# AndrewCullacino/handwritten-chinese-ocr-samples

Measured on AMD Instinct MI355X. Metric: text-lines/sec (1x128x2000 synth) greedy decode, higher is better.
Workload: dtype f16 (f32 accumulate); 1 GPU; BASELINE configs[1]: 64 x 1x128x2000 uint8 lines, random-init hctr checkpoint (C=7358), forward + greedy CTC decode, labels to host; global_lines=64, lines_per_gpu=64, width=2000, classes=7358, checkpoint=random, parallelism=batch-shard x1

## Files before the change

### handwritten-chinese-ocr-samples_amd/_lib.py

```python
import ctypes
import os
import subprocess
import sys

PKG_DIR = os.path.dirname(os.path.abspath(__file__))
ROOT = os.path.dirname(PKG_DIR)
CSRC = os.path.join(PKG_DIR, "csrc")
LIB_PATH = os.path.join(PKG_DIR, "libhctr_hip.so")
HEADER = os.path.join(ROOT, "include", "hctr_hip.h")

SOURCES = [("gather.cpp", ["-x", "hip"]), ("kernels.hip", []), ("preprocess.hip", ["-ffp-contract=off"]), ("engine.cpp", ["-x", "hip"]), ("beam_search.cpp", ["-ffp-contract=off"]),
           ("ngram_lm.cpp", ["-ffp-contract=off"])]
COMMON = ["--offload-arch=gfx950", "-O3", "-std=c++17", "-fPIC", "-Wall", "-Wno-unused-function"]

HCTR_OK = 0
ERR_ARG, ERR_HIP, ERR_STATE, ERR_KEY, ERR_SHAPE, ERR_EMPTY_LINE, ERR_NOMEM = -1, -2, -3, -4, -5, -6, -7
U8, F32, I64 = 0, 1, 2


def _headers():
    return [os.path.join(CSRC, "kernels.h"), os.path.join(CSRC, "ngram_lm.h"), os.path.join(CSRC, "lm_flat.h"), HEADER]


def _deps():
    return [os.path.join(CSRC, s) for s, _ in SOURCES] + _headers()


def source_hash():
    import hashlib
    h = hashlib.sha256()
    h.update(repr((COMMON, SOURCES)).encode())
    for d in sorted(_deps()):
        h.update(os.path.basename(d).encode())
        with open(d, "rb") as f:
            h.update(f.read())
    return h.hexdigest()[:16]


_MARK = b"hctr-src="


def embedded_hash(path=None):
    path = path or LIB_PATH
    try:
# ... 137 lines not shown
    ("hctr_nbest_skip_logits", _I, [_VP, _VP, _VP, _I, _I, _I, _I, _I, _I, ctypes.c_double, ctypes.c_double, _VP, _VP, _VP,
                                    _VP, _VP, _VP, _VP, _VP, _VP]),
    ("hctr_nbest_skip", _I, [_VP, _VP, _VP, _I, _I, _VP, _I, _I, _I, _I, ctypes.c_double, ctypes.c_double, _VP, _VP, _VP,
                             _VP, _VP, _VP, _VP, _VP, _VP]),
    ("hctr_beam_search", _I, [ctypes.POINTER(BeamParams), _I, _I, _I, _I, _VP, _VP, _VP, _VP, _VP, _VP, _VP,
                              _VP, _VP, _VP]),
    ("hctr_ngram_load", _I, [ctypes.c_char_p, ctypes.POINTER(_VP)]),
    ("hctr_ngram_free", None, [_VP]),
    ("hctr_ngram_order", _I, [_VP]),
    ("hctr_ngram_word_id", ctypes.c_int32, [_VP, ctypes.c_char_p]),
    ("hctr_ngram_score", ctypes.c_double, [_VP, ctypes.c_char_p, _I, _I]),
    ("hctr_ngram_word_logp", ctypes.c_double, [_VP, _VP, _I, ctypes.c_int32]),
    ("hctr_ngram_last_error", ctypes.c_char_p, []),
    ("hctr_comm_unique_id", _I, [_VP]),
    ("hctr_comm_create", _I, [ctypes.POINTER(_VP), _VP, _I, _I, _I]),
    ("hctr_comm_destroy", None, [_VP]),
    ("hctr_gather_labels", _I, [_VP, _VP, _VP, _I, _I, _I, _I, _VP, _VP]),
    ("hctr_comm_last_error", ctypes.c_char_p, []),
    ("hctr_resize_lines", _I, [_VP, _VP, _I64, c_i64p, c_i32p, c_i32p, c_i32p, _I, _I, c_i32p, _I, _VP, _I]),
    ("hctr_set_profiling", _I, [_VP, _I]),
    ("hctr_last_profile", _I, [_VP, ctypes.c_char_p, _I, c_f32p, _I]),
    ("hctr_debug_stamps", _I64, [_VP, ctypes.c_char_p, _VP, _I64]),
    ("hctr_debug_activation", _I64, [_VP, ctypes.c_char_p, _VP, _I64, ctypes.POINTER(_I), ctypes.POINTER(_I)]),
]


def load():
    global _LIB
    if _LIB is not None:
        return _LIB
    alt = os.environ.get("HCTR_LIB_PATH", "")
    if alt:
        if not os.path.isfile(alt):
            raise RuntimeError("HCTR_LIB_PATH=%s does not exist" % alt)
    elif _stale():
        try:
            build()
        except FileNotFoundError as exc:
            if not os.path.isfile(LIB_PATH):
                raise RuntimeError("libhctr_hip.so is missing and hipcc is not available (%s); "
                                   "the hctr engine has no CPU fallback" % exc)
            print("hctr: WARNING: sources are newer than libhctr_hip.so but hipcc is not available; "
                  "loading the prebuilt library", file=sys.stderr)
        except (OSError, subprocess.CalledProcessError) as exc:
            raise RuntimeError("libhctr_hip.so is out of date and rebuilding it failed (%s); fix the build "
                               "(python -c 'import hctr_amd; hctr_amd.build(force=True, verbose=True)')" % exc)
    try:
        import torch
    except ImportError:
        pass
    lib = ctypes.CDLL(alt or LIB_PATH)
    if not alt and embedded_hash() != source_hash():
        print("hctr: WARNING: libhctr_hip.so was built from other sources than csrc/ holds now (%s vs %s)"
              % (embedded_hash(), source_hash()), file=sys.stderr)
    host_only = bool(alt) and os.environ.get("HCTR_HOST_ONLY", "") == "1"
    for name, res, args in SIGNATURES:
        if host_only and not hasattr(lib, name):
            continue
        fn = getattr(lib, name)
        fn.restype = res
        fn.argtypes = args
    _LIB = lib
    return lib


_EXC = {ERR_ARG: ValueError, ERR_HIP: RuntimeError, ERR_STATE: RuntimeError, ERR_KEY: KeyError,
        ERR_SHAPE: RuntimeError, ERR_EMPTY_LINE: IndexError, ERR_NOMEM: MemoryError}


def check(rc, ctx=None):
    if rc == HCTR_OK:
        return
    msg = load().hctr_last_error(ctx)
    msg = msg.decode("utf-8", "replace") if msg else ""
    raise _EXC.get(rc, RuntimeError)("hctr engine error %d: %s" % (rc, msg))


def usable_cpus():
    n = len(os.sched_getaffinity(0))
    for path in ("/sys/fs/cgroup/cpu.max",):
        try:
# ... 16 lines not shown
```

### handwritten-chinese-ocr-samples_amd/csrc/engine.cpp

```cpp
#include "../../include/hctr_hip.h"
#include "kernels.h"

#include <algorithm>
#include <cfloat>
#include <cmath>
#include <cstdarg>
#include <cstdio>
#include <cstring>
#include <map>
#include <new>
#include <string>
#include <vector>

using namespace hctr;

namespace {

constexpr int kImgH = 128;
constexpr int kFeat = 2048;
constexpr double kBnEps = 1e-5;
constexpr int kStagePlanes[4] = {128, 256, 512, 512};
constexpr int kStageBlocks[4] = {2, 4, 5, 1};
constexpr int kStageH[5] = {128, 64, 32, 16, 8};
constexpr int64_t kDefaultMaxCols = 131072;

std::string g_create_error;

struct HostTensor {
    std::vector<float> data;
    std::vector<int64_t> shape;
    mutable bool used = false;
};

struct ConvW {
    half_t* w = nullptr;
    float* bias = nullptr;
    int cin = 0, cout = 0, coutPad = 0, taps = 0;
};

struct SeW {
    float* w1 = nullptr;
    float* w2 = nullptr;
    int c = 0;
};

struct BlockW {
    ConvW conv1, conv2, ds;
    SeW se;
    bool has_ds = false;
};

struct Workspace {
    int B = 0, W = 0, Wa = 0;
    void* img = nullptr;
    int32_t* widths = nullptr;
    half_t* s0 = nullptr;
    half_t* x[5] = {};
    half_t* p[5][3] = {};
// ... 258 lines not shown
                    const double v = (double)w->data[((size_t)co * cin + ci) * taps + t] * sc;
                    wmax = std::max(wmax, std::fabs(v));
                    half_t* row = &hw[((size_t)t * coutPad + blk * 64 + s) * cinp];
                    const half_t hi = (half_t)(float)v;
                    row[ci] = hi;
                    if (c->split) {
                        row[cin + ci] = hi;
                        row[2 * cin + ci] = (c->x3_mask & 1) ? (half_t)(float)(v - (double)(float)hi) : (half_t)0.f;
                    }
                }
        }
    for (int co = 0; co < cout; ++co) {
        const double sc = (double)g->data[co] / std::sqrt((double)var->data[co] + kBnEps);
        const double bb = has_bias ? (double)b->data[co] : 0.0;
        hb[co] = (float)((bb - (double)mean->data[co]) * sc + (double)beta->data[co]);
    }
    if (!(wmax < 65000.0))
        return fail(c, HCTR_ERR_ARG, "%s: BatchNorm-folded weight magnitude %.3g does not fit fp16", ck.c_str(), wmax);
    out->cin = cinp; out->cout = cout; out->coutPad = coutPad; out->taps = taps;
    TRY(dev_alloc(c, c->wallocs, &out->w, hw.size(), false));
    TRY(dev_alloc(c, c->wallocs, &out->bias, hb.size(), false));
    HIP_TRY(c, hipMemcpyAsync(out->w, hw.data(), hw.size() * sizeof(half_t), hipMemcpyHostToDevice, c->stream));
    HIP_TRY(c, hipMemcpyAsync(out->bias, hb.data(), hb.size() * sizeof(float), hipMemcpyHostToDevice, c->stream));
    HIP_TRY(c, hipStreamSynchronize(c->stream));
    return HCTR_OK;
}

int build_se(hctr_ctx* c, const std::string& key, int ch, SeW* out) {
    const HostTensor *w1, *w2;
    TRY(need(c, key + ".fc.0.weight", {ch / 16, ch}, &w1));
    TRY(need(c, key + ".fc.2.weight", {ch, ch / 16}, &w2));
    out->c = ch;
    TRY(dev_alloc(c, c->wallocs, &out->w1, w1->data.size(), false));
    TRY(dev_alloc(c, c->wallocs, &out->w2, w2->data.size(), false));
    HIP_TRY(c, hipMemcpyAsync(out->w1, w1->data.data(), w1->data.size() * 4, hipMemcpyHostToDevice, c->stream));
    HIP_TRY(c, hipMemcpyAsync(out->w2, w2->data.data(), w2->data.size() * 4, hipMemcpyHostToDevice, c->stream));
    HIP_TRY(c, hipStreamSynchronize(c->stream));
    return HCTR_OK;
}

int build_stem(hctr_ctx* c, WeightSet& ws) {
    const HostTensor *w, *b, *g, *beta, *mean, *var;
    TRY(need(c, "cnn.conv0_1.weight", {64, 1, 3, 3}, &w));
    TRY(need(c, "cnn.conv0_1.bias", {64}, &b));
    TRY(need(c, "cnn.bn0_1.weight", {64}, &g));
    TRY(need(c, "cnn.bn0_1.bias", {64}, &beta));
// ... 222 lines not shown
    if (c->profiling) { c->prof.clear(); c->ev_used = 0; }
    c->h_widths.clear();
}

struct ActDesc {
    half_t* p;
    int H, C;
};

ConvTile pick_tile(const hctr_ctx* c, const ConvW& cw, int H) {
    if (cw.cout == 64) return TILE_64x256;
    if (c->halo_mode == 2 && cw.taps == 9 && cw.coutPad % 128 == 0 && H % 16 == 0) return TILE_HALO4;
    if (c->halo_mode == 2 && cw.taps == 9 && cw.coutPad % 128 == 0 && H % 8 == 0) return TILE_HALO4_8x32;
    if (c->big_tiles && cw.coutPad % 256 == 0 && H % 16 == 0) return TILE_256x256;
    return TILE_128x128;
}

int run_conv(hctr_ctx* c, Prof& pf, const char* name, const ConvW& cw, ActDesc in, half_t* out, int outH,
             bool relu, bool pool, float* se_part, bool to_head, const float* se_scale = nullptr,
             const half_t* resid = nullptr, const ConvW* ds = nullptr, const half_t* ds_in = nullptr,
             int stem_img_f32 = -1, bool stem_widths = false) {
    const Workspace& ws = c->ws;
    ConvArgs a{};
    a.x = in.p; a.w = cw.w; a.bias = cw.bias; a.y = out; a.se_part = se_part;
    a.se_scale = se_scale; a.resid = resid;
    a.split = c->split ? 1 : 0;
    a.drop_lo = (c->split && !(c->x3_mask & c->out_class)) ? 1 : 0;
    const int m = c->chm();
    a.H = in.H; a.W = ws.W; a.Cin = cw.cin; a.Cout = cw.cout; a.CoutPad = cw.coutPad;
    const ConvTile tile = pick_tile(c, cw, in.H);
    const int rows = conv_tile_rows(tile);
    if (in.H % rows != 0 || cw.cin % kBK != 0)
        return fail(c, HCTR_ERR_ARG, "conv %s: H=%d or Cin=%d not tileable", name, in.H, cw.cin);
    const int cols = conv_tile_cols(tile);
    a.tilesW = (ws.W + cols - 1) / cols;
    a.tilesH = in.H / rows;
    a.in_sb = (int64_t)(in.H + 2) * ws.Wa * cw.cin;
    a.in_sh = ws.Wa * cw.cin;
    if (a.in_sb * 2 >= ((int64_t)1 << 32) || (int64_t)(outH + 2) * ws.Wa * cw.cout * m * 2 >= ((int64_t)1 << 32))
        return fail(c, HCTR_ERR_ARG, "line width %d too large: one image's activation exceeds the kernels' 32-bit "
                    "in-image byte offsets (conv %s)", ws.W, name);
    if (to_head) {
        a.out_sb = (int64_t)ws.W * kFeat * m; a.out_sh = 512 * m; a.out_sw = kFeat * m; a.out_off = 0;
        a.out_wlimit = ws.W;
    } else {
        a.out_sb = (int64_t)(outH + 2) * ws.Wa * cw.cout * m;
        a.out_sh = ws.Wa * cw.cout * m; a.out_sw = cw.cout * m;
// ... 2314 lines not shown
            } else {
                L.mode = 2;
            }
        }
        HIP_TRY(c, hipSetDevice(c->device));
        std::vector<void*> tmp;
        PoolGuard tmp_guard{tmp};
        return synced(c, [&]() -> int {
            uint8_t *src = nullptr, *dst = out;
            ResizeLine* dl = nullptr;
            const size_t out_bytes = (size_t)n * out_height * out_W;
            TRY(dev_alloc(c, tmp, &src, (size_t)std::max<int64_t>(packed_bytes, 1), false));
            TRY(dev_alloc(c, tmp, &dl, (size_t)n, false));
            if (!out_on_device) TRY(dev_alloc(c, tmp, &dst, out_bytes, false));
            HIP_TRY(c, hipMemcpyAsync(src, packed_src, (size_t)packed_bytes, hipMemcpyHostToDevice, c->stream));
            HIP_TRY(c, hipMemcpyAsync(dl, lines.data(), sizeof(ResizeLine) * (size_t)n, hipMemcpyHostToDevice, c->stream));
            HIP_TRY(c, launch_resize_lines(src, dl, n, dst, out_height, out_W, c->stream));
            if (!out_on_device) HIP_TRY(c, hipMemcpyAsync(out, dst, out_bytes, hipMemcpyDeviceToHost, c->stream));
            return HCTR_OK;
        }());
    });
}

int64_t hctr_debug_stamps(hctr_ctx* c, const char* layer, uint64_t* out, int64_t cap_wgs) {
    return guard<int64_t>(c, [&]() -> int64_t {
        if (!c || cap_wgs < 0) return HCTR_ERR_ARG;
        if (hipSetDevice(c->device) != hipSuccess) return fail(c, HCTR_ERR_HIP, "hipSetDevice");
        if (layer) {
            if (c->stamp_buf) { (void)hipFree(c->stamp_buf); c->stamp_buf = nullptr; }
            c->stamp_layer = layer;
            c->stamp_cap = cap_wgs;
            c->stamp_n = 0;
            if (cap_wgs > 0 && hipMalloc((void**)&c->stamp_buf, (size_t)cap_wgs * 128) != hipSuccess)
                return fail(c, HCTR_ERR_NOMEM, "stamp buffer");
            return 0;
        }
        if (!out || !c->stamp_buf) return fail(c, HCTR_ERR_STATE, "stamping not armed");
        const int64_t n = std::min(c->stamp_n, cap_wgs);
        if (hipMemcpy(out, c->stamp_buf, (size_t)n * 128, hipMemcpyDeviceToHost) != hipSuccess)
            return fail(c, HCTR_ERR_HIP, "stamp copy");
        return n;
    });
}

int64_t hctr_debug_activation(hctr_ctx* c, const char* name, float* out, int64_t cap, int* Cout, int* Hout) {
    return guard<int64_t>(c, [&]() -> int64_t {
// ... 50 lines not shown
```

### handwritten-chinese-ocr-samples_amd/csrc/kernels.h

```cpp
#pragma once
#include <hip/hip_runtime.h>
#include <stdint.h>

#include "lm_flat.h"

namespace hctr {

typedef _Float16 half_t;

constexpr int kTileW = 16;
constexpr int kBK = 64;

struct ConvArgs {
    const half_t* x;
    const half_t* w;
    const float* bias;
    void* y;
    float* se_part;
    const float* se_scale;
    const half_t* resid;
    int H, W;
    int Cin, Cout, CoutPad;
    int tilesW, tilesH;
    int64_t in_sb;
    int in_sh;
    int64_t out_sb;
    int out_sh, out_sw;
    int64_t out_off;
    int out_wlimit;
    int relu, pool;
    int64_t M;
    int64_t ldo;
    int mtiles, ntiles;
    int nt_shift, th_shift;
    uint64_t tw_magic;
    float* amax_val;
    int32_t* amax_idx;
    float* amax_val2;
// ... 187 lines not shown
```

### handwritten-chinese-ocr-samples_amd/csrc/kernels.hip

```cpp
#include "kernels.h"

#include <algorithm>
#include <cstdlib>

namespace hctr {

typedef _Float16 f16x8 __attribute__((ext_vector_type(8)));
typedef float f32x4 __attribute__((ext_vector_type(4)));
typedef float f32x2 __attribute__((ext_vector_type(2)));
typedef _Float16 f16x2 __attribute__((ext_vector_type(2)));
typedef uint32_t u32x4 __attribute__((ext_vector_type(4)));
typedef void __attribute__((address_space(3))) * lptr_t;

__device__ __forceinline__ void glds16_asm(const char* gsrc, char* lds_dst) {
    const uint32_t lds = (uint32_t)(uintptr_t)((lptr_t)lds_dst);
    uint32_t keep;
    asm volatile("s_mov_b32 %0, m0\n\ts_mov_b32 m0, %2\n\ts_nop 0\n\tglobal_load_lds_dwordx4 %1, off\n\ts_mov_b32 m0, %0"
                 : "=&s"(keep)
                 : "v"(gsrc), "s"(lds)
                 : "memory");
}

template <int CTRL>
__device__ __forceinline__ float dpp_f32(float v) {
// ... 6 lines not shown
__device__ __forceinline__ void glds16_asm_s(const char* sbase, uint32_t voff, char* lds_dst) {
    const uint32_t lds = (uint32_t)(uintptr_t)((lptr_t)lds_dst);
    uint32_t keep;
    asm volatile("s_mov_b32 %0, m0\n\ts_mov_b32 m0, %3\n\ts_nop 0\n\tglobal_load_lds_dwordx4 %1, %2\n\ts_mov_b32 m0, %0"
                 : "=&s"(keep)
                 : "v"(voff), "s"(sbase), "s"(lds)
                 : "memory");
}

__device__ __forceinline__ void glds16x4_asm_s(const char* s0, const char* s1, const char* s2, const char* s3, uint32_t voff,
                                               char* d0, char* d1, char* d2, char* d3) {
    const uint32_t l0 = (uint32_t)(uintptr_t)((lptr_t)d0), l1 = (uint32_t)(uintptr_t)((lptr_t)d1);
    const uint32_t l2 = (uint32_t)(uintptr_t)((lptr_t)d2), l3 = (uint32_t)(uintptr_t)((lptr_t)d3);
    uint32_t keep;
    asm volatile("s_mov_b32 %0, m0\n\t"
                 "s_mov_b32 m0, %6\n\ts_nop 0\n\tglobal_load_lds_dwordx4 %1, %2\n\t"
                 "s_mov_b32 m0, %7\n\ts_nop 0\n\tglobal_load_lds_dwordx4 %1, %3\n\t"
                 "s_mov_b32 m0, %8\n\ts_nop 0\n\tglobal_load_lds_dwordx4 %1, %4\n\t"
                 "s_mov_b32 m0, %9\n\ts_nop 0\n\tglobal_load_lds_dwordx4 %1, %5\n\t"
                 "s_mov_b32 m0, %0"
                 : "=&s"(keep)
                 : "v"(voff), "s"(s0), "s"(s1), "s"(s2), "s"(s3), "s"(l0), "s"(l1), "s"(l2), "s"(l3)
                 : "memory");
}

template <int LSTRIDE>
__device__ __forceinline__ void glds16x4v_asm_s(const char* sbase, uint32_t v0, uint32_t v1, uint32_t v2, uint32_t v3, char* d0) {
    const uint32_t l0 = (uint32_t)(uintptr_t)((lptr_t)d0);
    uint32_t keep;
    asm volatile("s_mov_b32 %0, m0\n\t"
                 "s_mov_b32 m0, %6\n\ts_nop 0\n\tglobal_load_lds_dwordx4 %1, %5\n\t"
                 "s_add_u32 m0, m0, %7\n\ts_nop 0\n\tglobal_load_lds_dwordx4 %2, %5\n\t"
                 "s_add_u32 m0, m0, %7\n\ts_nop 0\n\tglobal_load_lds_dwordx4 %3, %5\n\t"
                 "s_add_u32 m0, m0, %7\n\ts_nop 0\n\tglobal_load_lds_dwordx4 %4, %5\n\t"
                 "s_mov_b32 m0, %0"
                 : "=&s"(keep)
                 : "v"(v0), "v"(v1), "v"(v2), "v"(v3), "s"(sbase), "s"(l0), "i"(LSTRIDE)
                 : "memory", "scc");
}

__device__ __forceinline__ constexpr int acc_cout_offset(int j) { return (j >> 2) * 64 + ((j >> 1) & 1) * 32 + (j & 1) * 4; }

constexpr float kSeScaleFloor = 1e-12f;

template <int WN, int WM, int JT, bool LINEAR, bool SPLIT, bool PRIVATE_RED = false, bool BIAS_DONE = false,
          bool RESID_IN_ACC = false>
// ... 754 lines not shown
                if (g + 2 < 8) read_a(g + 2, ar[(g + 2) % 3]);
                __builtin_amdgcn_sched_barrier(0);
                if (g == 1) { read_b(1, bq[1]); __builtin_amdgcn_sched_barrier(0); }
                __builtin_amdgcn_s_setprio(1);
#pragma unroll
                for (int jj = 0; jj < 2; ++jj)
#pragma unroll
                    for (int n = 0; n < 4; ++n)
                        acc[2 * jp + jj][n] = __builtin_amdgcn_mfma_f32_16x16x32_f16(ar[g % 3][jj], bq[ks][n],
                                                                                    acc[2 * jp + jj][n], 0, 0, 0);
                __builtin_amdgcn_s_setprio(0);
                __builtin_amdgcn_sched_barrier(0);
            }
        }
    }
    asm volatile("s_waitcnt vmcnt(0)" ::: "memory");
    conv_epilogue<WN, WM, JT, false, false>(a, acc, smem, tid, lane, wn, wm, n0, mt, img, th, tw, th * 16 + wm * 4,
                                            tw * 16);
}

namespace halo4_lds {
constexpr int kWeightBuf = 16384;
constexpr int kWeights = 0;
constexpr int kHalo = kWeights + 2 * kWeightBuf;
constexpr int kScratch = kHalo + kHaloBytes;
constexpr int kScratchBytes = 4 * 128 * 4;
constexpr int kHaloTable = kScratch;
constexpr int kHaloTableBytes = 4 * 12 * 8 * 4;
constexpr int kNextTile = kScratch + kScratchBytes;
constexpr int kTotal = kNextTile + 16;
static_assert(kHaloTableBytes <= kScratchBytes, "the halo-offset table fits inside the epilogue scratch it aliases");
static_assert(kNextTile >= kScratch + kScratchBytes, "the next-tile words lie behind the epilogue scratch");
static_assert(kTotal <= 80 * 1024, "two workgroups per CU on 160 KB of LDS");
}

template <int GEOM, bool SPLIT, bool PERSIST, bool STAMP = false, bool DSFUSE = false, bool RESPRE = false>
__global__ __launch_bounds__(256, 2) void conv3x3_halo4_kernel(const ConvArgs a) {
    static_assert(!DSFUSE || !PERSIST, "downsample fusion: non-persistent instances only");
    static_assert(!RESPRE || (!DSFUSE && !PERSIST && !SPLIT), "residual-in-prologue: plain f16 instances only");
    constexpr int WN = 1, WM = 4, JT = 8, BN = 128;
    constexpr int TR = GEOM ? 8 : 16, TC = GEOM ? 32 : 16;
    constexpr int S = TC + 4;
    static_assert((TR + 2) * S * 128 == kHaloBytes, "halo footprint");
    extern __shared__ __attribute__((aligned(16))) char smem[];
    const int tid = threadIdx.x;
    auto stamp = [&](int i) {
        if (STAMP && tid == 0) a.stamps[(size_t)blockIdx.x * 16 + i] = __builtin_amdgcn_s_memrealtime();
    };
    stamp(0);
    const int lane = tid & 63;
    const int wv = __builtin_amdgcn_readfirstlane(tid >> 6);
    const int wm = wv;
    const int cin = a.Cin;
    const int nkc = (a.dbg & 64) ? 0 : cin / kBK;
    const int nk = 9 * nkc;
    constexpr bool kPrefetch = !PERSIST && !STAMP && !RESPRE;
    static_assert(!(kPrefetch && PERSIST), "the halo-offset table aliases the epilogue scratch: one tile per workgroup");
    constexpr int kRing = 3;
    constexpr int kBhalfAt = 1;
    constexpr int kBpreAt = 4;
    constexpr int kEarlyAt = 1;

    {
        const int k0 = a.mtiles, k1 = a.ntiles, k2 = a.tilesW, k3 = a.tilesH, k4 = a.Cin, k5 = a.in_sh, k6 = a.nt_shift,
                  k7 = a.th_shift, k8 = a.CoutPad;
        const uint64_t k9 = a.tw_magic;
        const int64_t k10 = a.in_sb;
        const half_t *k11 = a.x, *k12 = a.w;
        const float* k13 = a.bias;
        asm volatile("" ::"s"(k0), "s"(k1), "s"(k2), "s"(k3), "s"(k4), "s"(k5), "s"(k6), "s"(k7), "s"(k8), "s"(k9), "s"(k10),
                     "s"(k11), "s"(k12), "s"(k13));
    }
    const int total = a.mtiles * a.ntiles;
    const int xcd = blockIdx.x & 7, local = blockIdx.x >> 3;
    const int tq = total >> 3, tr = total & 7;
    const int xbase_lin = xcd < tr ? xcd * (tq + 1) : tr * (tq + 1) + (xcd - tr) * tq;
    const int xcnt = tq + (xcd < tr ? 1 : 0);
    const int nloc = PERSIST ? (int)(gridDim.x >> 3) : 1;
    struct Tile { int n0, mt, img, th, tw; const char* xb; const char* wb; };
    auto tile_at = [&](int idx) {
        Tile t;
        const int lin = xbase_lin + idx;
        int nt, t2, th, img;
        if (a.nt_shift >= 0) { nt = lin & (a.ntiles - 1); t.mt = lin >> a.nt_shift; }
        else { nt = lin % a.ntiles; t.mt = lin / a.ntiles; }
        t.n0 = nt * BN;
        t2 = (int)(((uint64_t)(uint32_t)t.mt * a.tw_magic) >> 40);
        const int tw = t.mt - t2 * a.tilesW;
        if (a.th_shift >= 0) { th = t2 & (a.tilesH - 1); img = t2 >> a.th_shift; }
        else { th = t2 % a.tilesH; img = t2 / a.tilesH; }
        t.img = img; t.th = th; t.tw = tw;
// ... 52 lines not shown
        uint32_t* htab = (uint32_t*)(smem + halo4_lds::kHaloTable);
        if ((lane & 7) == 0) {
            const uint32_t cp0 = (uint32_t)((lane >> 3) & 7) << 4;
#pragma unroll
            for (int r = 0; r < 12; ++r) htab[(wv * 12 + r) * 8 + (lane >> 3)] = hoff[r] - cp0;
        }
    };
    const int hbuf = halo4_lds::kHalo + wrow * (S * 128);
    int bx[3][2];
#pragma unroll
    for (int d = 0; d < 3; ++d) {
        const int u = wcol + c + d;
        const int v0 = u * 128 + (((q ^ (u & 7)) & 7) << 4);
        bx[d][0] = hbuf + v0;
        bx[d][1] = hbuf + (v0 ^ 64);
    }
    auto b_ptrs = [&](int tap, const char*& be, const char*& bo) {
        const int tdy = tap / 3, d = tap - tdy * 3;
        be = smem + bx[d][tdy & 1] + tdy * (S * 128);
        bo = smem + bx[d][(tdy & 1) ^ 1] + tdy * (S * 128);
    };

    Tile cur = tile_at(tidx);
    int kbase = 0;
    bool first = true;

    int tile_no = 0;
    for (;;) {
        const bool has_next = PERSIST && (tnext < xcnt);
        const char* nxb = cur.xb;
        const char* nwb = cur.wb;
        if (has_next) {
            const Tile t = tile_at(tnext);
            nxb = t.xb;
            nwb = t.wb;
        }
        int drawn = 0;
        if (dynamic && tid == 0)
            drawn = 2 * nloc + __hip_atomic_fetch_add(a.tile_counter + xcd, 1, __ATOMIC_RELAXED, __HIP_MEMORY_SCOPE_AGENT);
        f32x4 acc[JT][4];
        f16x8 bq[2][4];
        auto mma_step = [&](const char* wt, const char* be, const char* bo, auto&& stage_next, auto&& after_group,
                            bool have_b0 = false, const char* nbe = nullptr, const char* nbo = nullptr,
                            int bhalf_at = kBhalfAt) {
            f16x8 ar[kRing][2];
            auto read_a = [&](int g, f16x8 (&dst)[2]) {
                const int ks = g >> 2, jp = g & 3;
                const char* base = wt + (ks ? aoff1 : aoff0);
                dst[0] = *(const f16x8*)(base + (2 * jp) * 2048);
                dst[1] = *(const f16x8*)(base + (2 * jp + 1) * 2048);
            };
            auto read_b = [&](int ks, f16x8 (&dst)[4]) {
#pragma unroll
                for (int n = 0; n < 4; ++n)
                    dst[n] = *(const f16x8*)((((n & 1) ^ ks) ? bo : be) + n * (S * 128));
            };
            __builtin_amdgcn_sched_barrier(0);
            if (!have_b0) read_b(0, bq[0]);
            read_a(0, ar[0]);
            __builtin_amdgcn_sched_barrier(0);
#pragma unroll
            for (int g = 1; g < kRing - 1; ++g) read_a(g, ar[g]);
            __builtin_amdgcn_sched_barrier(0);
            stage_next();
            __builtin_amdgcn_sched_barrier(0);
#pragma unroll
            for (int g = 0; g < 8; ++g) {
                const int ks = g >> 2, jp = g & 3;
                if (g + kRing - 1 < 8) read_a(g + kRing - 1, ar[(g + kRing - 1) % kRing]);
                __builtin_amdgcn_sched_barrier(0);
                if (g == bhalf_at) { read_b(1, bq[1]); __builtin_amdgcn_sched_barrier(0); }
#pragma unroll
                for (int jj = 0; jj < 2; ++jj)
#pragma unroll
                    for (int n = 0; n < 4; ++n)
                        acc[2 * jp + jj][n] = __builtin_amdgcn_mfma_f32_16x16x32_f16(
                            ar[g % kRing][jj], bq[ks][n], acc[2 * jp + jj][n], 0, 0, 0);
                if (g == kBpreAt && nbe != nullptr) {
#pragma unroll
                    for (int n = 0; n < 4; ++n) bq[0][n] = *(const f16x8*)(((n & 1) ? nbo : nbe) + n * (S * 128));
                }
                after_group(g);
                __builtin_amdgcn_sched_barrier(0);
            }
        };

        if (DSFUSE) {
            const int dcin = a.ds_cin, nds = dcin / kBK;
            const int tw0 = cur.tw, th0 = cur.th, img0 = cur.img;
            const char* dxb = (const char*)(a.ds_x + img0 * a.ds_in_sb + (int64_t)(th0 * TR) * a.ds_in_sh +
                                            (int64_t)(tw0 * TC) * dcin);
            const char* dwb = (const char*)(a.ds_w + (int64_t)cur.n0 * dcin);
            uint32_t woff_x[4];
            lane_offsets(dcin, a.ds_in_sh, woff_x, true);
            lane_offsets(cin, a.in_sh, woff, false);
            stage_halo(dxb, 0);
            stage_w(dwb, dcin, woff_x, 0, 0, 0);
            __builtin_amdgcn_s_setprio(1);
#pragma unroll
            for (int j = 0; j < JT; ++j)
#pragma unroll
                for (int n = 0; n < 4; ++n) acc[j][n] = (f32x4){0.f, 0.f, 0.f, 0.f};
            __builtin_amdgcn_s_waitcnt(0xc07f);
#pragma unroll 1
            for (int kc = 0; kc < nds; ++kc) {
                asm volatile("s_waitcnt vmcnt(0)" ::: "memory");
                __builtin_amdgcn_s_barrier();
                asm volatile("" ::: "memory");
                const char *be, *bo;
                b_ptrs(4, be, bo);
                mma_step(weight_buf(kc), be, bo, [&] {
                    if (kc + 1 < nds) stage_w(dwb, dcin, woff_x, kc + 1, 0, (kc + 1) & 1);
                    else stage_w(cur.wb, cin, woff, 0, 0, (kc + 1) & 1);
                }, [&](int) {});
                __builtin_amdgcn_s_barrier();
                asm volatile("" ::: "memory");
                if (kc + 1 < nds) {
                    stage_halo(dxb, kc + 1);
                } else {
                    lane_offsets(cin, a.in_sh, woff, true);
                    stage_halo(cur.xb, 0);
                    if (kPrefetch) write_halo_table();
                }
            }
            kbase = nds;
            const float* sc = a.se_scale + (int64_t)img0 * a.Cout + cur.n0 + q * 8;
#pragma unroll
            for (int j = 0; j < JT; ++j) {
                const int o = acc_cout_offset(j);
                const f32x4 bd = *(const f32x4*)(a.ds_bias + cur.n0 + q * 8 + o);
                const f32x4 b2 = *(const f32x4*)(a.bias + cur.n0 + q * 8 + o);
                const f32x4 s4 = *(const f32x4*)(sc + o);
#pragma unroll
                for (int i = 0; i < 4; ++i) {
                    const float inv = __builtin_amdgcn_rcpf(fmaxf(s4[i], kSeScaleFloor));
#pragma unroll
                    for (int n = 0; n < 4; ++n) acc[j][n][i] = fmaf(acc[j][n][i] + bd[i], inv, b2[i]);
                }
            }
        } else {
            if (PERSIST || first) lane_offsets(cin, a.in_sh, woff, true);
            if (first) {
                stage_halo(cur.xb, 0);
                stage_weights(cur.wb, 0, 0, 0);
                if (kPrefetch) write_halo_table();
                first = false;
                if (STAMP) {
                    stamp(1);
                    asm volatile("s_waitcnt vmcnt(0)" ::: "memory");
                    __builtin_amdgcn_s_barrier();
                    stamp(2);
                }
            }
            if (RESPRE) {
                const int w = cur.tw * TC + wcol + c;
                const bool wok = w < a.out_wlimit;
                const half_t* rb = a.resid + a.out_off + cur.img * a.out_sb + (int64_t)w * a.out_sw + cur.n0 + q * 8 +
                                   (int64_t)(cur.th * TR + wrow) * a.out_sh;
                const float* sc = a.se_scale + (int64_t)cur.img * a.Cout + cur.n0 + q * 8;
                f16x8 rlo[JT / 4][4], rhi[JT / 4][4];
#pragma unroll
                for (int cb = 0; cb < JT / 4; ++cb)
#pragma unroll
                    for (int n = 0; n < 4; ++n) {
                        const half_t* r = rb + (int64_t)n * a.out_sh + cb * 64;
                        rlo[cb][n] = wok ? *(const f16x8*)r : (f16x8){0, 0, 0, 0, 0, 0, 0, 0};
                        rhi[cb][n] = wok ? *(const f16x8*)(r + 32) : (f16x8){0, 0, 0, 0, 0, 0, 0, 0};
// ... 5 lines not shown
#pragma unroll
                    for (int i = 0; i < 4; ++i) {
                        const float inv = __builtin_amdgcn_rcpf(fmaxf(s4[i], kSeScaleFloor));
                        const int e = (j & 3) * 4 + i;
#pragma unroll
                        for (int n = 0; n < 4; ++n) {
                            const float r = e < 8 ? (float)rlo[j >> 2][n][e] : (float)rhi[j >> 2][n][e - 8];
                            acc[j][n][i] = fmaf(r, inv, b4[i]);
                        }
                    }
                }
            } else {
#pragma unroll
                for (int j = 0; j < JT; ++j) {
                    const f32x4 b4 = *(const f32x4*)(a.bias + cur.n0 + q * 8 + acc_cout_offset(j));
#pragma unroll
                    for (int n = 0; n < 4; ++n) acc[j][n] = b4;
                }
            }
        }

        __builtin_amdgcn_s_waitcnt(0xc07f);
        __builtin_amdgcn_s_setprio(1);
        for (int kc = 0; kc < nkc; ++kc) {
            const bool next_chunk = kc + 1 < nkc;
#pragma unroll
            for (int tap = 0; tap < 9; ++tap) {
                const int k = kc * 9 + tap;
                asm volatile("s_waitcnt vmcnt(0)" ::: "memory");
                if (!(a.dbg & 1024)) __builtin_amdgcn_s_barrier();
                asm volatile("" ::: "memory");
                const char *be, *bo;
                b_ptrs(tap, be, bo);
                const bool more = k + 1 < nk;
                const bool wrap = tap == 8;
                const int tap1 = more ? (wrap ? 0 : tap + 1) : 0;
                const int kc1 = more ? (wrap ? kc + 1 : kc) : 0;
                const char* wsrc = more ? cur.wb : nwb;
                const char *nbe = nullptr, *nbo = nullptr;
                if (kPrefetch && tap < 8) b_ptrs(tap + 1, nbe, nbo);
                mma_step(weight_buf(kbase + k), be, bo, [&] {
                    if ((more || has_next) && !(a.dbg & 512))
                        stage_weights(wsrc, kc1, tap1, (kbase + k + 1) & 1);
                }, [&](int g) {
                    if (kPrefetch && tap == 8 && g == kEarlyAt && next_chunk) {
                        asm volatile("s_waitcnt lgkmcnt(0)" ::: "memory");
                        __builtin_amdgcn_s_barrier();
                        asm volatile("" ::: "memory");
                        static_assert(kHaloPieces == 45, "halo piece count");
                        const char* hsrc = (next_chunk ? cur.xb + (int64_t)(kc + 1) * (kBK * 2) : nxb);
                        char* d = smem + halo4_lds::kHalo + wv * 1024;
                        int ln = lane;
                        asm volatile("" : "+v"(ln));
                        const uint32_t* hrow = (const uint32_t*)(smem + halo4_lds::kHaloTable) + wv * 96 + (ln >> 3);
                        const uint32_t cpl = (uint32_t)((ln ^ (ln >> 3)) & 7) << 4;
                        uint32_t ho[4];
#pragma unroll
                        for (int r = 0; r < 4; ++r) ho[r] = hrow[r * 8] + cpl;
                        glds16x4v_asm_s<4096>(hsrc, ho[0], ho[1], ho[2], ho[3], d);
#pragma unroll
                        for (int r = 0; r < 4; ++r) ho[r] = hrow[(4 + r) * 8] + cpl;
                        glds16x4v_asm_s<4096>(hsrc, ho[0], ho[1], ho[2], ho[3], d + 4 * 4096);
#pragma unroll
                        for (int r = 0; r < 4; ++r) ho[r] = hrow[(8 + r) * 8] + cpl;
#pragma unroll
                        for (int r = 8; r < 11; ++r) glds16_asm_s(hsrc, ho[r - 8], d + r * 4096);
                        if (wv == 0) glds16_asm_s(hsrc, ho[3], d + 11 * 4096);
                    }
                }, kPrefetch && tap > 0, nbe, nbo, (kPrefetch && tap == 8) ? 0 : kBhalfAt);
            }
            if (!kPrefetch && (next_chunk || has_next) && !(a.dbg & 32)) {
                __builtin_amdgcn_s_barrier();
                asm volatile("" ::: "memory");
                if (next_chunk) stage_halo(cur.xb, kc + 1);
                else stage_halo(nxb, 0);
            }
        }
        __builtin_amdgcn_s_setprio(0);
        stamp(3);
        if (a.dbg & 128) {
            float t = 0.f;
#pragma unroll
            for (int j = 0; j < JT; ++j)
#pragma unroll
                for (int n = 0; n < 4; ++n) t += acc[j][n][0] + acc[j][n][1] + acc[j][n][2] + acc[j][n][3];
            if (t == 123.456f) ((half_t*)a.y)[0] = (half_t)t;
        } else
        {
            const int tw = cur.tw, th = cur.th, img = cur.img;
            conv_epilogue<WN, WM, JT, false, SPLIT, true, true, DSFUSE || RESPRE>(
                a, acc, smem + halo4_lds::kScratch, tid, lane, 0, wm, cur.n0, cur.mt, img, th, tw, th * TR + wrow,
                tw * TC + wcol, STAMP ? a.stamps + (size_t)blockIdx.x * 16 : nullptr);
        }
        if (!has_next) break;
// ... 187 lines not shown
            }
        }
    }
    __builtin_amdgcn_s_setprio(0);
    conv_epilogue<WN, WM, JT, false, false, true, true, false>(a, acc, smem + halo4_lds::kScratch, tid, lane, 0, wm, n0, mt, img, th, tw,
                                                               th * TR + wrow, tw * TC + wcol);
}

template <auto KERNEL>
static hipError_t launch_halo4_instance(const ConvArgs& a0, int grid, hipStream_t s, bool with_env_dbg = true) {
    static bool done[64] = {};
    hipError_t e0 = raise_lds_limit((const void*)KERNEL, halo4_lds::kTotal, done);
    if (e0 != hipSuccess) return e0;
    static const int dbg = env_dbg();
    ConvArgs a = a0;
    if (with_env_dbg) a.dbg |= dbg;
    hipLaunchKernelGGL(KERNEL, dim3(grid), dim3(256), halo4_lds::kTotal, s, a);
    return hipGetLastError();
}

template <int GEOM, bool SPLIT, bool PERSIST>
static hipError_t launch_conv_halo4_tp(const ConvArgs& a, hipStream_t s) {
    int grid = a.mtiles * a.ntiles;
    if (PERSIST) {
        static int cus[64] = {};
        int dev = 0;
        (void)hipGetDevice(&dev);
        if (dev >= 0 && dev < 64 && cus[dev] == 0) {
            hipDeviceProp_t prop;
            if (hipGetDeviceProperties(&prop, dev) == hipSuccess) cus[dev] = prop.multiProcessorCount;
            if (cus[dev] <= 0) cus[dev] = 256;
        }
        const int resident = 2 * ((dev >= 0 && dev < 64) ? cus[dev] : 256);
        if (grid > resident) grid = resident;
        grid = (grid + 7) / 8 * 8;
    }
    return launch_halo4_instance<conv3x3_halo4_kernel<GEOM, SPLIT, PERSIST>>(a, grid, s);
}
template <int GEOM, bool SPLIT>
static hipError_t launch_conv_halo4_t(const ConvArgs& a, hipStream_t s) {
    const int grid = a.mtiles * a.ntiles;
    if (a.ds_x != nullptr) {
        if (GEOM != 0) return hipErrorInvalidValue;
        return launch_halo4_instance<conv3x3_halo4_kernel<0, SPLIT, false, false, true>>(a, grid, s);
    }
    if (a.stamps != nullptr && !SPLIT)
        return launch_halo4_instance<conv3x3_halo4_kernel<GEOM, false, false, true>>(a, grid, s, false);
    static const int persist = [] { const char* e = getenv("HCTR_PERSIST"); return e ? atoi(e) : 0; }();
    if constexpr (!SPLIT) {
        static const int respre = [] { const char* e = getenv("HCTR_RESPRE"); return e ? atoi(e) : 0; }();
        if (respre && persist == 0 && a.resid != nullptr && a.se_scale != nullptr)
            return launch_halo4_instance<conv3x3_halo4_kernel<GEOM, false, false, false, false, true>>(a, grid, s);
    }
    if (persist == 0 || (persist == 2 && a.tile_counter == nullptr)) return launch_conv_halo4_tp<GEOM, SPLIT, false>(a, s);
    ConvArgs b = a;
    if (persist != 2) b.tile_counter = nullptr;
    return launch_conv_halo4_tp<GEOM, SPLIT, true>(b, s);
}
template <int GEOM>
static hipError_t launch_conv_halo4(const ConvArgs& a0, hipStream_t s) {
    ConvArgs a = a0;
    auto shift_of = [](int v) { int sft = 0; while ((1 << sft) < v) ++sft; return (1 << sft) == v ? sft : -1; };
    a.nt_shift = shift_of(a.ntiles);
    a.th_shift = shift_of(a.tilesH);
    if (a.tilesW < 1 || (uint64_t)a.mtiles * (uint64_t)a.tilesW >= ((uint64_t)1 << 40)) return hipErrorInvalidValue;
    a.tw_magic = (((uint64_t)1 << 40) + (uint64_t)a.tilesW - 1) / (uint64_t)a.tilesW;
// ... 2853 lines not shown
```

### include/hctr_hip.h

```cpp
#ifndef HCTR_HIP_H
#define HCTR_HIP_H

#include <stdint.h>

#ifdef __cplusplus
extern "C" {
#endif

typedef struct hctr_ctx hctr_ctx;

typedef enum {
    HCTR_OK = 0,
    HCTR_ERR_ARG = -1,
    HCTR_ERR_HIP = -2,
    HCTR_ERR_STATE = -3,
    HCTR_ERR_KEY = -4,
    HCTR_ERR_SHAPE = -5,
    HCTR_ERR_EMPTY_LINE = -6,
    HCTR_ERR_NOMEM = -7
} hctr_status;

typedef enum { HCTR_U8 = 0, HCTR_F32 = 1, HCTR_I64 = 2 } hctr_dtype;

int hctr_create(hctr_ctx** out, int device, int num_classes);
// ... 164 lines not shown

int hctr_resize_lines(hctr_ctx* ctx, const uint8_t* packed_src, int64_t packed_bytes, const int64_t* offsets,
                      const int32_t* heights, const int32_t* widths, const int32_t* channels, int n,
                      int out_height, const int32_t* out_widths, int out_W, uint8_t* out, int out_on_device);

#define HCTR_COMM_ID_BYTES 128
typedef struct hctr_comm hctr_comm;
int hctr_comm_unique_id(void* id128);
int hctr_comm_create(hctr_comm** out, const void* id128, int rank, int world, int device);
void hctr_comm_destroy(hctr_comm* comm);
int hctr_gather_labels(hctr_comm* comm, const int32_t* labels, const int32_t* lengths, int n_local, int row_stride,
                       int lines_per_rank, int cap, int32_t* out_labels, int32_t* out_lengths);
const char* hctr_comm_last_error(void);

int hctr_set_profiling(hctr_ctx* ctx, int enabled);
int hctr_last_profile(hctr_ctx* ctx, char* names_buf, int cap, float* ms, int max_n);
int hctr_workspace_stats(hctr_ctx* ctx, int64_t* arena_bytes, int64_t* arena_allocations, int64_t* recarves);
int hctr_lines_per_pass(hctr_ctx* ctx, int B, int W, int f16x3);
int64_t hctr_debug_stamps(hctr_ctx* ctx, const char* layer, uint64_t* out, int64_t cap_wgs);

int64_t hctr_debug_activation(hctr_ctx* ctx, const char* name, float* out, int64_t cap,
                              int* C, int* H);

#ifdef __cplusplus
}
#endif
#endif
```

Before: 524.9 lines/s.

## Pre-pack 3x3 conv weights into MFMA-order stream with 4-slot LDS ring

Adds a host-side repack of 3x3 conv weights into a lane-ordered stream layout matching the MFMA operand fragments. The non-persistent halo4 conv kernel can then stage weights with contiguous global_load_lds copies into a four-slot LDS ring, issuing half-tap units at two points per step. This replaces the strided per-lane weight staging and its offset math, and should allow finer-grained overlap of weight loads with MFMA work. The cost is a second device copy of every 3x3 weight. Launches now fail if the packed weights are missing, and the prefetch path is split into a separate loop.

New measurement: 529.3 lines/s, median of 6. Within noise of the previous version (+0.8%).

```diff
diff --git a/handwritten-chinese-ocr-samples_amd/_lib.py b/handwritten-chinese-ocr-samples_amd/_lib.py
--- a/handwritten-chinese-ocr-samples_amd/_lib.py
+++ b/handwritten-chinese-ocr-samples_amd/_lib.py
@@ -19,7 +19,8 @@
 
 
 def _headers():
-    return [os.path.join(CSRC, "kernels.h"), os.path.join(CSRC, "ngram_lm.h"), os.path.join(CSRC, "lm_flat.h"), HEADER]
+    return [os.path.join(CSRC, "kernels.h"), os.path.join(CSRC, "ngram_lm.h"), os.path.join(CSRC, "lm_flat.h"),
+            os.path.join(CSRC, "weight_stream.h"), HEADER]
 
 
 def _deps():
@@ -203,6 +204,7 @@
     ("hctr_last_profile", _I, [_VP, ctypes.c_char_p, _I, c_f32p, _I]),
     ("hctr_debug_stamps", _I64, [_VP, ctypes.c_char_p, _VP, _I64]),
     ("hctr_debug_activation", _I64, [_VP, ctypes.c_char_p, _VP, _I64, ctypes.POINTER(_I), ctypes.POINTER(_I)]),
+    ("hctr_pack_weight_stream", _I, [_VP, _VP, _I, _I, _I, _I]),
 ]
 
 
@@ -238,6 +240,8 @@
     for name, res, args in SIGNATURES:
         if host_only and not hasattr(lib, name):
             continue
+        if alt and name == "hctr_pack_weight_stream" and not hasattr(lib, name):
+            continue
         fn = getattr(lib, name)
         fn.restype = res
         fn.argtypes = args
diff --git a/handwritten-chinese-ocr-samples_amd/csrc/engine.cpp b/handwritten-chinese-ocr-samples_amd/csrc/engine.cpp
--- a/handwritten-chinese-ocr-samples_amd/csrc/engine.cpp
+++ b/handwritten-chinese-ocr-samples_amd/csrc/engine.cpp
@@ -1,5 +1,6 @@
 #include "../../include/hctr_hip.h"
 #include "kernels.h"
+#include "weight_stream.h"
 
 #include <algorithm>
 #include <cfloat>
@@ -34,6 +35,7 @@
 
 struct ConvW {
     half_t* w = nullptr;
+    half_t* ws = nullptr;
     float* bias = nullptr;
     int cin = 0, cout = 0, coutPad = 0, taps = 0;
 };
@@ -338,6 +340,14 @@
     TRY(dev_alloc(c, c->wallocs, &out->bias, hb.size(), false));
     HIP_TRY(c, hipMemcpyAsync(out->w, hw.data(), hw.size() * sizeof(half_t), hipMemcpyHostToDevice, c->stream));
     HIP_TRY(c, hipMemcpyAsync(out->bias, hb.data(), hb.size() * sizeof(float), hipMemcpyHostToDevice, c->stream));
+    std::vector<half_t> hs;
+    if (taps == 9 && wstream::shape_ok(taps, coutPad, cinp)) {
+        static_assert(sizeof(half_t) == sizeof(uint16_t), "fp16 storage");
+        hs.resize(hw.size());
+        wstream::pack((const uint16_t*)hw.data(), (uint16_t*)hs.data(), taps, coutPad, cinp, false);
+        TRY(dev_alloc(c, c->wallocs, &out->ws, hs.size(), false));
+        HIP_TRY(c, hipMemcpyAsync(out->ws, hs.data(), hs.size() * sizeof(half_t), hipMemcpyHostToDevice, c->stream));
+    }
     HIP_TRY(c, hipStreamSynchronize(c->stream));
     return HCTR_OK;
 }
@@ -606,7 +616,7 @@
              int stem_img_f32 = -1, bool stem_widths = false) {
     const Workspace& ws = c->ws;
     ConvArgs a{};
-    a.x = in.p; a.w = cw.w; a.bias = cw.bias; a.y = out; a.se_part = se_part;
+    a.x = in.p; a.w = cw.w; a.ws = cw.ws; a.bias = cw.bias; a.y = out; a.se_part = se_part;
     a.se_scale = se_scale; a.resid = resid;
     a.split = c->split ? 1 : 0;
     a.drop_lo = (c->split && !(c->x3_mask & c->out_class)) ? 1 : 0;
@@ -2967,6 +2977,12 @@
     });
 }
 
+int hctr_pack_weight_stream(const uint16_t* src, uint16_t* dst, int taps, int coutPad, int cin, int inverse) {
+    if (!src || !dst || !wstream::shape_ok(taps, coutPad, cin)) return HCTR_ERR_ARG;
+    wstream::pack(src, dst, taps, coutPad, cin, inverse != 0);
+    return HCTR_OK;
+}
+
 int64_t hctr_debug_stamps(hctr_ctx* c, const char* layer, uint64_t* out, int64_t cap_wgs) {
     return guard<int64_t>(c, [&]() -> int64_t {
         if (!c || cap_wgs < 0) return HCTR_ERR_ARG;
diff --git a/handwritten-chinese-ocr-samples_amd/csrc/kernels.h b/handwritten-chinese-ocr-samples_amd/csrc/kernels.h
--- a/handwritten-chinese-ocr-samples_amd/csrc/kernels.h
+++ b/handwritten-chinese-ocr-samples_amd/csrc/kernels.h
@@ -14,6 +14,7 @@
 struct ConvArgs {
     const half_t* x;
     const half_t* w;
+    const half_t* ws;
     const float* bias;
     void* y;
     float* se_part;
diff --git a/handwritten-chinese-ocr-samples_amd/csrc/kernels.hip b/handwritten-chinese-ocr-samples_amd/csrc/kernels.hip
--- a/handwritten-chinese-ocr-samples_amd/csrc/kernels.hip
+++ b/handwritten-chinese-ocr-samples_amd/csrc/kernels.hip
@@ -52,6 +52,19 @@
                  : "=&s"(keep)
                  : "v"(voff), "s"(s0), "s"(s1), "s"(s2), "s"(s3), "s"(l0), "s"(l1), "s"(l2), "s"(l3)
                  : "memory");
+}
+
+__device__ __forceinline__ void glds16x2_asm_s(const char* s0, uint32_t voff, char* d0) {
+    const char* s1 = s0 + 1024;
+    const uint32_t l0 = (uint32_t)(uintptr_t)((lptr_t)d0);
+    uint32_t keep;
+    asm volatile("s_mov_b32 %0, m0\n\t"
+                 "s_mov_b32 m0, %4\n\ts_nop 0\n\tglobal_load_lds_dwordx4 %1, %2\n\t"
+                 "s_add_u32 m0, m0, 1024\n\ts_nop 0\n\tglobal_load_lds_dwordx4 %1, %3\n\t"
+                 "s_mov_b32 m0, %0"
+                 : "=&s"(keep)
+                 : "v"(voff), "s"(s0), "s"(s1), "s"(l0)
+                 : "memory", "scc");
 }
 
 template <int LSTRIDE>
@@ -852,6 +865,9 @@
 namespace halo4_lds {
 constexpr int kWeightBuf = 16384;
 constexpr int kWeights = 0;
+constexpr int kRingSlot = 8192, kRingSlots = 4;
+static_assert(kRingSlots * kRingSlot == 2 * kWeightBuf, "the ring slots are the two weight buffers");
+static_assert(kRingSlot == 8 * 64 * 16, "a unit is eight 16-cout blocks of 64 lanes x 16 bytes");
 constexpr int kHalo = kWeights + 2 * kWeightBuf;
 constexpr int kScratch = kHalo + kHaloBytes;
 constexpr int kScratchBytes = 4 * 128 * 4;
@@ -886,6 +902,7 @@
     const int nk = 9 * nkc;
     constexpr bool kPrefetch = !PERSIST && !STAMP && !RESPRE;
     static_assert(!(kPrefetch && PERSIST), "the halo-offset table aliases the epilogue scratch: one tile per workgroup");
+    constexpr bool kRingW = kPrefetch;
     constexpr int kRing = 3;
     constexpr int kBhalfAt = 1;
     constexpr int kBpreAt = 4;
@@ -896,7 +913,7 @@
                   k7 = a.th_shift, k8 = a.CoutPad;
         const uint64_t k9 = a.tw_magic;
         const int64_t k10 = a.in_sb;
-        const half_t *k11 = a.x, *k12 = a.w;
+        const half_t *k11 = a.x, *k12 = kRingW ? a.ws : a.w;
         const float* k13 = a.bias;
         asm volatile("" ::"s"(k0), "s"(k1), "s"(k2), "s"(k3), "s"(k4), "s"(k5), "s"(k6), "s"(k7), "s"(k8), "s"(k9), "s"(k10),
                      "s"(k11), "s"(k12), "s"(k13));
@@ -995,6 +1012,10 @@
     };
 
     Tile cur = tile_at(tidx);
+    const char* const wsb = kRingW ? (const char*)(a.ws + (int64_t)cur.n0 * 9 * cin) + wv * 2048 : nullptr;
+    char* const wl = smem + halo4_lds::kWeights + wv * 2048;
+    const uint32_t l16 = (uint32_t)lane * 16u;
+    auto stage_unit = [&](const char* src, int slot_off) { glds16x2_asm_s(src, l16, wl + slot_off); };
     int kbase = 0;
     bool first = true;
 
@@ -1013,9 +1034,7 @@
             drawn = 2 * nloc + __hip_atomic_fetch_add(a.tile_counter + xcd, 1, __ATOMIC_RELAXED, __HIP_MEMORY_SCOPE_AGENT);
         f32x4 acc[JT][4];
         f16x8 bq[2][4];
-        auto mma_step = [&](const char* wt, const char* be, const char* bo, auto&& stage_next, auto&& after_group,
-                            bool have_b0 = false, const char* nbe = nullptr, const char* nbo = nullptr,
-                            int bhalf_at = kBhalfAt) {
+        auto mma_step = [&](const char* wt, const char* be, const char* bo, auto&& stage_next) {
             f16x8 ar[kRing][2];
             auto read_a = [&](int g, f16x8 (&dst)[2]) {
                 const int ks = g >> 2, jp = g & 3;
@@ -1029,13 +1048,51 @@
                     dst[n] = *(const f16x8*)((((n & 1) ^ ks) ? bo : be) + n * (S * 128));
             };
             __builtin_amdgcn_sched_barrier(0);
+            read_b(0, bq[0]);
+            read_a(0, ar[0]);
+            __builtin_amdgcn_sched_barrier(0);
+#pragma unroll
+            for (int g = 1; g < kRing - 1; ++g) read_a(g, ar[g]);
+            __builtin_amdgcn_sched_barrier(0);
+            stage_next();
+            __builtin_amdgcn_sched_barrier(0);
+#pragma unroll
+            for (int g = 0; g < 8; ++g) {
+                const int ks = g >> 2, jp = g & 3;
+                if (g + kRing - 1 < 8) read_a(g + kRing - 1, ar[(g + kRing - 1) % kRing]);
+                __builtin_amdgcn_sched_barrier(0);
+                if (g == kBhalfAt) { read_b(1, bq[1]); __builtin_amdgcn_sched_barrier(0); }
+#pragma unroll
+                for (int jj = 0; jj < 2; ++jj)
+#pragma unroll
+                    for (int n = 0; n < 4; ++n)
+                        acc[2 * jp + jj][n] = __builtin_amdgcn_mfma_f32_16x16x32_f16(
+                            ar[g % kRing][jj], bq[ks][n], acc[2 * jp + jj][n], 0, 0, 0);
+                __builtin_amdgcn_sched_barrier(0);
+            }
+        };
+        auto ring_step = [&](const char* wt, const char* be, const char* bo, auto&& issue0, auto&& mid, auto&& issue1,
+                             auto&& after_group, bool have_b0, const char* nbe, const char* nbo, int bhalf_at) {
+            f16x8 ar[kRing][2];
+            auto read_a = [&](int g, f16x8 (&dst)[2]) {
+                const int ks = g >> 2, jp = g & 3;
+                const char* base = wt + ks * halo4_lds::kRingSlot;
+                dst[0] = *(const f16x8*)(base + (2 * jp) * 1024);
+                dst[1] = *(const f16x8*)(base + (2 * jp + 1) * 1024);
+            };
+            auto read_b = [&](int ks, f16x8 (&dst)[4]) {
+#pragma unroll
+                for (int n = 0; n < 4; ++n)
+                    dst[n] = *(const f16x8*)((((n & 1) ^ ks) ? bo : be) + n * (S * 128));
+            };
+            __builtin_amdgcn_sched_barrier(0);
             if (!have_b0) read_b(0, bq[0]);
             read_a(0, ar[0]);
             __builtin_amdgcn_sched_barrier(0);
 #pragma unroll
             for (int g = 1; g < kRing - 1; ++g) read_a(g, ar[g]);
             __builtin_amdgcn_sched_barrier(0);
-            stage_next();
+            issue0();
             __builtin_amdgcn_sched_barrier(0);
 #pragma unroll
             for (int g = 0; g < 8; ++g) {
@@ -1055,6 +1112,11 @@
                 }
                 after_group(g);
                 __builtin_amdgcn_sched_barrier(0);
+                if (g == 3) {
+                    mid();
+                    issue1();
+                    __builtin_amdgcn_sched_barrier(0);
+                }
             }
         };
 
@@ -1065,8 +1127,8 @@
                                             (int64_t)(tw0 * TC) * dcin);
             const char* dwb = (const char*)(a.ds_w + (int64_t)cur.n0 * dcin);
             uint32_t woff_x[4];
+            static_assert(!DSFUSE || kRingW, "the fused downsample hands over to the ring loop");
             lane_offsets(dcin, a.ds_in_sh, woff_x, true);
-            lane_offsets(cin, a.in_sh, woff, false);
             stage_halo(dxb, 0);
             stage_w(dwb, dcin, woff_x, 0, 0, 0);
             __builtin_amdgcn_s_setprio(1);
@@ -1084,8 +1146,11 @@
                 b_ptrs(4, be, bo);
                 mma_step(weight_buf(kc), be, bo, [&] {
                     if (kc + 1 < nds) stage_w(dwb, dcin, woff_x, kc + 1, 0, (kc + 1) & 1);
-                    else stage_w(cur.wb, cin, woff, 0, 0, (kc + 1) & 1);
-                }, [&](int) {});
+                    else {
+                        stage_unit(wsb, (nds & 1) * halo4_lds::kWeightBuf);
+                        stage_unit(wsb + halo4_lds::kRingSlot, (nds & 1) * halo4_lds::kWeightBuf + halo4_lds::kRingSlot);
+                    }
+                });
                 __builtin_amdgcn_s_barrier();
                 asm volatile("" ::: "memory");
                 if (kc + 1 < nds) {
@@ -1115,7 +1180,12 @@
             if (PERSIST || first) lane_offsets(cin, a.in_sh, woff, true);
             if (first) {
                 stage_halo(cur.xb, 0);
-                stage_weights(cur.wb, 0, 0, 0);
+                if (kRingW) {
+                    stage_unit(wsb, 0);
+                    stage_unit(wsb + halo4_lds::kRingSlot, halo4_lds::kRingSlot);
+                } else {
+                    stage_weights(cur.wb, 0, 0, 0);
+                }
                 if (kPrefetch) write_halo_table();
                 first = false;
                 if (STAMP) {
@@ -1167,6 +1237,62 @@
 
         __builtin_amdgcn_s_waitcnt(0xc07f);
         __builtin_amdgcn_s_setprio(1);
+        if constexpr (kRingW) {
+            const int ub = DSFUSE ? (a.ds_cin / kBK) & 1 : 0;
+            stage_unit(wsb + 2 * halo4_lds::kRingSlot, (ub ^ 1) * halo4_lds::kWeightBuf);
+            const char* const wlane = smem + halo4_lds::kWeights + l16;
+            for (int kc = 0; kc < nkc; ++kc) {
+                const bool next_chunk = kc + 1 < nkc;
+                const int pe = ((kc + ub) & 1) * halo4_lds::kWeightBuf, po = halo4_lds::kWeightBuf - pe;
+                const char* const csrc = wsb + (int64_t)kc * (18 * halo4_lds::kRingSlot);
+#pragma unroll
+                for (int tap = 0; tap < 9; ++tap) {
+                    const int pt = (tap & 1) ? po : pe, pn = (tap & 1) ? pe : po;
+                    if (tap == 8 && !next_chunk) asm volatile("s_waitcnt vmcnt(0)" ::: "memory");
+                    else asm volatile("s_waitcnt vmcnt(2)" ::: "memory");
+                    __builtin_amdgcn_s_barrier();
+                    asm volatile("" ::: "memory");
+                    const char *be, *bo, *nbe = nullptr, *nbo = nullptr;
+                    b_ptrs(tap, be, bo);
+                    if (tap < 8) b_ptrs(tap + 1, nbe, nbo);
+                    ring_step(wlane + pt, be, bo, [&] {
+                        if (tap < 8 || next_chunk)
+                            stage_unit(csrc + (2 * tap + 3) * halo4_lds::kRingSlot, pn + halo4_lds::kRingSlot);
+                    }, [&] {
+                        __builtin_amdgcn_s_barrier();
+                        asm volatile("" ::: "memory");
+                    }, [&] {
+                        if (tap < 7 || next_chunk)
+                            stage_unit(csrc + (2 * tap + 4) * halo4_lds::kRingSlot, pt);
+                    }, [&](int g) {
+                        if (tap == 8 && g == kEarlyAt && next_chunk) {
+                            asm volatile("s_waitcnt lgkmcnt(0)" ::: "memory");
+                            __builtin_amdgcn_s_barrier();
+                            asm volatile("" ::: "memory");
+                            static_assert(kHaloPieces == 45, "halo piece count");
+                            const char* hsrc = cur.xb + (int64_t)(kc + 1) * (kBK * 2);
+                            char* d = smem + halo4_lds::kHalo + wv * 1024;
+                            int ln = lane;
+                            asm volatile("" : "+v"(ln));
+                            const uint32_t* hrow = (const uint32_t*)(smem + halo4_lds::kHaloTable) + wv * 96 + (ln >> 3);
+                            const uint32_t cpl = (uint32_t)((ln ^ (ln >> 3)) & 7) << 4;
+                            uint32_t ho[4];
+#pragma unroll
+                            for (int r = 0; r < 4; ++r) ho[r] = hrow[r * 8] + cpl;
+                            glds16x4v_asm_s<4096>(hsrc, ho[0], ho[1], ho[2], ho[3], d);
+#pragma unroll
+                            for (int r = 0; r < 4; ++r) ho[r] = hrow[(4 + r) * 8] + cpl;
+                            glds16x4v_asm_s<4096>(hsrc, ho[0], ho[1], ho[2], ho[3], d + 4 * 4096);
+#pragma unroll
+                            for (int r = 0; r < 4; ++r) ho[r] = hrow[(8 + r) * 8] + cpl;
+#pragma unroll
+                            for (int r = 8; r < 11; ++r) glds16_asm_s(hsrc, ho[r - 8], d + r * 4096);
+                            if (wv == 0) glds16_asm_s(hsrc, ho[3], d + 11 * 4096);
+                        }
+                    }, tap > 0, nbe, nbo, tap == 8 ? 0 : kBhalfAt);
+                }
+            }
+        } else
         for (int kc = 0; kc < nkc; ++kc) {
             const bool next_chunk = kc + 1 < nkc;
 #pragma unroll
@@ -1182,39 +1308,12 @@
                 const int tap1 = more ? (wrap ? 0 : tap + 1) : 0;
                 const int kc1 = more ? (wrap ? kc + 1 : kc) : 0;
                 const char* wsrc = more ? cur.wb : nwb;
-                const char *nbe = nullptr, *nbo = nullptr;
-                if (kPrefetch && tap < 8) b_ptrs(tap + 1, nbe, nbo);
                 mma_step(weight_buf(kbase + k), be, bo, [&] {
                     if ((more || has_next) && !(a.dbg & 512))
                         stage_weights(wsrc, kc1, tap1, (kbase + k + 1) & 1);
-                }, [&](int g) {
-                    if (kPrefetch && tap == 8 && g == kEarlyAt && next_chunk) {
-                        asm volatile("s_waitcnt lgkmcnt(0)" ::: "memory");
-                        __builtin_amdgcn_s_barrier();
-                        asm volatile("" ::: "memory");
-                        static_assert(kHaloPieces == 45, "halo piece count");
-                        const char* hsrc = (next_chunk ? cur.xb + (int64_t)(kc + 1) * (kBK * 2) : nxb);
-                        char* d = smem + halo4_lds::kHalo + wv * 1024;
-                        int ln = lane;
-                        asm volatile("" : "+v"(ln));
-                        const uint32_t* hrow = (const uint32_t*)(smem + halo4_lds::kHaloTable) + wv * 96 + (ln >> 3);
-                        const uint32_t cpl = (uint32_t)((ln ^ (ln >> 3)) & 7) << 4;
-                        uint32_t ho[4];
-#pragma unroll
-                        for (int r = 0; r < 4; ++r) ho[r] = hrow[r * 8] + cpl;
-                        glds16x4v_asm_s<4096>(hsrc, ho[0], ho[1], ho[2], ho[3], d);
-#pragma unroll
-                        for (int r = 0; r < 4; ++r) ho[r] = hrow[(4 + r) * 8] + cpl;
-                        glds16x4v_asm_s<4096>(hsrc, ho[0], ho[1], ho[2], ho[3], d + 4 * 4096);
-#pragma unroll
-                        for (int r = 0; r < 4; ++r) ho[r] = hrow[(8 + r) * 8] + cpl;
-#pragma unroll
-                        for (int r = 8; r < 11; ++r) glds16_asm_s(hsrc, ho[r - 8], d + r * 4096);
-                        if (wv == 0) glds16_asm_s(hsrc, ho[3], d + 11 * 4096);
-                    }
-                }, kPrefetch && tap > 0, nbe, nbo, (kPrefetch && tap == 8) ? 0 : kBhalfAt);
-            }
-            if (!kPrefetch && (next_chunk || has_next) && !(a.dbg & 32)) {
+                });
+            }
+            if ((next_chunk || has_next) && !(a.dbg & 32)) {
                 __builtin_amdgcn_s_barrier();
                 asm volatile("" ::: "memory");
                 if (next_chunk) stage_halo(cur.xb, kc + 1);
@@ -1448,6 +1547,7 @@
 template <int GEOM, bool SPLIT, bool PERSIST>
 static hipError_t launch_conv_halo4_tp(const ConvArgs& a, hipStream_t s) {
     int grid = a.mtiles * a.ntiles;
+    if (!PERSIST && a.ws == nullptr) return hipErrorInvalidValue;
     if (PERSIST) {
         static int cus[64] = {};
         int dev = 0;
@@ -1467,7 +1567,7 @@
 static hipError_t launch_conv_halo4_t(const ConvArgs& a, hipStream_t s) {
     const int grid = a.mtiles * a.ntiles;
     if (a.ds_x != nullptr) {
-        if (GEOM != 0) return hipErrorInvalidValue;
+        if (GEOM != 0 || a.ws == nullptr) return hipErrorInvalidValue;
         return launch_halo4_instance<conv3x3_halo4_kernel<0, SPLIT, false, false, true>>(a, grid, s);
     }
     if (a.stamps != nullptr && !SPLIT)
diff --git a/handwritten-chinese-ocr-samples_amd/csrc/weight_stream.h b/handwritten-chinese-ocr-samples_amd/csrc/weight_stream.h
--- /dev/null
+++ b/handwritten-chinese-ocr-samples_amd/csrc/weight_stream.h
@@ -0,0 +1,36 @@
+#pragma once
+#include <cstddef>
+#include <cstdint>
+
+namespace wstream {
+
+constexpr int kTileCouts = 128, kChunk = 64;
+
+inline bool shape_ok(int taps, int coutPad, int cin) {
+    return taps > 0 && coutPad > 0 && cin > 0 && coutPad % kTileCouts == 0 && cin % kChunk == 0;
+}
+
+inline size_t row_index(size_t s, int taps, int coutPad, int cin) {
+    const int e = (int)(s & 7), lane = (int)((s >> 3) & 63), j = (int)((s >> 9) & 7), ks = (int)((s >> 12) & 1);
+    size_t u = s >> 13;
+    const int tap = (int)(u % (size_t)taps);
+    u /= (size_t)taps;
+    const int nkc = cin / kChunk;
+    const int kc = (int)(u % (size_t)nkc), tile = (int)(u / (size_t)nkc);
+    const int row = tile * kTileCouts + j * 16 + (lane & 15);
+    const int col = kc * kChunk + ks * 32 + (lane >> 4) * 8 + e;
+    return ((size_t)tap * coutPad + row) * cin + col;
+}
+
+inline void pack(const uint16_t* src, uint16_t* dst, int taps, int coutPad, int cin, bool inverse) {
+    const size_t n = (size_t)taps * coutPad * cin;
+    for (size_t s0 = 0; s0 < n; s0 += 8) {
+        const size_t r0 = row_index(s0, taps, coutPad, cin);
+        for (int e = 0; e < 8; ++e) {
+            if (inverse) dst[r0 + e] = src[s0 + e];
+            else dst[s0 + e] = src[r0 + e];
+        }
+    }
+}
+
+}
diff --git a/include/hctr_hip.h b/include/hctr_hip.h
--- a/include/hctr_hip.h
+++ b/include/hctr_hip.h
@@ -210,6 +210,8 @@
 int64_t hctr_debug_activation(hctr_ctx* ctx, const char* name, float* out, int64_t cap,
                               int* C, int* H);
 
+int hctr_pack_weight_stream(const uint16_t* src, uint16_t* dst, int taps, int coutPad, int cin, int inverse);
+
 #ifdef __cplusplus
 }
 #endif
```
